# YoungYoung619/road-object-detection-for-bdd100k

Measured on AMD Instinct MI355X. Metric: training images/sec at 1280x720 bf16, higher is better.
Workload: dtype bf16; 1 GPU; REFINE train step (train.py), MobileNet-v2 RefineDet, 720x1280, 8 images/GPU; global_batch=8, train_range=REFINE, parallelism=dp1, augment=False, hip_graph=True, graph_mode=full

## Files before the change

road-object-detection-for-bdd100k_amd/csrc/gemm.hip:

```cpp
#include "rod_common.h"
#include "bnstat_common.h"

namespace rod {

constexpr int BK = 32;

template <typename T> struct LdsPad;
template <> struct LdsPad<bf16_t> { static constexpr int v = 8; };
template <> struct LdsPad<float> { static constexpr int v = 4; };

template <typename T> struct Chunk8;
template <> struct Chunk8<bf16_t> {
  bf16x8 v;
  bool ok;
  __device__ __forceinline__ void zero() {
#pragma unroll
    for (int j = 0; j < 8; ++j) v[j] = (bf16_t)0.f;
    ok = false;
  }
  __device__ __forceinline__ void load_vec(const bf16_t* p) {
    v = *(const bf16x8*)p;
    ok = true;
  }
  __device__ __forceinline__ void set(int j, bf16_t x) { v[j] = x; }
// ... 1218 lines not shown
    __syncthreads();
  }
  const int K = KS * KS * Cin;
  const int tid = threadIdx.x, lane = tid & 63, wave = tid >> 6;
  const int wm = wave >> 1, wn = wave & 1;
  int tile = blockIdx.x, split = blockIdx.y;
  if (gridDim.x > 1 && (gridDim.y & 7) == 0) {
    const long pl = blockIdx.x + (long)blockIdx.y * gridDim.x;
    const long q = pl >> 3;
    tile = (int)(q % gridDim.x);
    split = (int)((q / gridDim.x) * 8 + (pl & 7));
  }
  const int co0 = (tile / ktiles) * WG_T;
  const int k0 = (tile % ktiles) * WG_T;
  const long mb = (long)split * chunk;
  const long me = mb + chunk < M ? mb + chunk : M;

  const int lr = tid >> 3;
  const int lc = (tid & 7) * 8;

  f32x4 acc[2][2];
#pragma unroll
  for (int a = 0; a < 2; ++a)
#pragma unroll
    for (int b = 0; b < 2; ++b)
#pragma unroll
      for (int r = 0; r < 4; ++r) acc[a][b][r] = 0.f;

  Chunk8<T> rdv[RPT], rxv[RPT];
  constexpr bool WALKW = KS == 3 && VA && CIN == 0;
  int wy[RPT], wx[RPT], wnn[RPT], kdy = 0, kdx = 0, kci = 0;
  bool kok = false;
  if constexpr (WALKW) {
    const int kk = k0 + lc;
    kok = kk < K;
    const int tap = kok ? kk / Cin : 0;
    kci = kk - tap * Cin;
    kdy = tap / 3 - 1;
    kdx = tap % 3 - 1;
#pragma unroll
    for (int u = 0; u < RPT; ++u) {
      const long row = mb + lr + u * BK;
      wx[u] = (int)(row % W);
      const long t = row / W;
      wy[u] = (int)(t % H);
      wnn[u] = (int)(t / H);
    }
  }
  auto load_one = [&](long row, Chunk8<T>& rd, Chunk8<T>& rx) {
    if (row >= me || co0 + lc >= Cout) {
      rd.zero();
    } else if (VD && co0 + lc + 8 <= Cout) {
      rd.load_vec(DY + row * lddy + co0 + lc);
    } else {
#pragma unroll
      for (int j = 0; j < 8; ++j) rd.set(j, (co0 + lc + j < Cout) ? DY[row * lddy + co0 + lc + j] : (T)0.f);
    }
    if constexpr (!WALKW) {
      RowSrc<T, KS, CIN> rs;
      rs.init(X, row < me ? row : M, M, H, W, ldx);
      rs.template load<VA, PRO>(rx, k0 + lc, K, Cin, H, W, ldx, pro_lds, pro.act);
    }
  };
  auto load_step = [&](long m) {
#pragma unroll
    for (int u = 0; u < RPT; ++u) {
      load_one(m + lr + u * BK, rdv[u], rxv[u]);
      if constexpr (WALKW) {
        const long row = m + lr + u * BK;
        const int yy = wy[u] + kdy, xx = wx[u] + kdx;
        if (kok && row < me && yy >= 0 && yy < H && xx >= 0 && xx < W)
          rxv[u].load_vec(X + (((long)wnn[u] * H + yy) * W + xx) * ldx + kci);
        else
          rxv[u].zero();
        wx[u] += RPT * BK;
        while (wx[u] >= W) {
          wx[u] -= W;
          if (++wy[u] == H) {
            wy[u] = 0;
            ++wnn[u];
          }
        }
      }
    }
  };

  if (mb < me) load_step(mb);
  for (long m = mb; m < me; m += RPT * BK) {
    __syncthreads();
#pragma unroll
    for (int u = 0; u < RPT; ++u) {
      rdv[u].store_lds(Ds + (lr + u * BK) * WG_LD + lc);
      if constexpr (PRO && WALKW) {
        if (rxv[u].ok) rxv[u].pro(pro_lds, kci, pro.act);
      } else if constexpr (PRO) {
        RowSrc<T, KS, CIN> rp;
        rp.template pro_pending<PRO>(rxv[u], k0 + lc, Cin, pro_lds, pro.act);
      }
      rxv[u].store_lds(Xs + (lr + u * BK) * WG_LD + lc);
    }
    __syncthreads();
    if (m + RPT * BK < me) load_step(m + RPT * BK);
#pragma unroll
    for (int u = 0; u < RPT; ++u)
    if constexpr (sizeof(T) == 2) {
      const int g = lane >> 4, i = lane & 15, q = i >> 2, p = i & 3;
#pragma unroll
      for (int a = 0; a < 2; ++a) {
        const int cb = wm * 32 + a * 16;
        const bf16x4 lo = tr_read((const bf16_t*)Ds + (u * BK + 8 * g + q) * WG_LD + cb + 4 * p);
        const bf16x4 hi = tr_read((const bf16_t*)Ds + (u * BK + 8 * g + 4 + q) * WG_LD + cb + 4 * p);
        bf16x8 fa = {lo[0], lo[1], lo[2], lo[3], hi[0], hi[1], hi[2], hi[3]};
#pragma unroll
        for (int b = 0; b < 2; ++b) {
          const int kb = wn * 32 + b * 16;
          const bf16x4 l2 = tr_read((const bf16_t*)Xs + (u * BK + 8 * g + q) * WG_LD + kb + 4 * p);
          const bf16x4 h2 = tr_read((const bf16_t*)Xs + (u * BK + 8 * g + 4 + q) * WG_LD + kb + 4 * p);
          bf16x8 fb = {l2[0], l2[1], l2[2], l2[3], h2[0], h2[1], h2[2], h2[3]};
          acc[a][b] = __builtin_amdgcn_mfma_f32_16x16x32_bf16(fa, fb, acc[a][b], 0, 0, 0);
        }
      }
    } else {
      const int i = lane & 15, q = lane >> 4;
#pragma unroll
      for (int kk = 0; kk < BK / 4; ++kk) {
        const int mr = u * BK + kk * 4 + q;
#pragma unroll
        for (int a = 0; a < 2; ++a) {
          const float av = ((const float*)Ds)[mr * WG_LD + wm * 32 + a * 16 + i];
#pragma unroll
          for (int b = 0; b < 2; ++b) {
            const float bv = ((const float*)Xs)[mr * WG_LD + wn * 32 + b * 16 + i];
            acc[a][b] = __builtin_amdgcn_mfma_f32_16x16x4f32(av, bv, acc[a][b], 0, 0, 0);
          }
        }
      }
    }
  }
  float* out = part + (long)split * Cout * K;
#pragma unroll
  for (int a = 0; a < 2; ++a)
#pragma unroll
    for (int b = 0; b < 2; ++b) {
      const int k = k0 + wn * 32 + b * 16 + (lane & 15);
      if (k >= K) continue;
#pragma unroll
      for (int r = 0; r < 4; ++r) {
        const int co = co0 + wm * 32 + a * 16 + (lane >> 4) * 4 + r;
        if (co < Cout) out[(long)co * K + k] = acc[a][b][r];
      }
    }
}


struct StemWgradPlan {
  int xb, yb, rb, nblk;
};
static StemWgradPlan stem_wgrad_plan(int N, int H, int W) {
  StemWgradPlan p;
  p.xb = cdiv(W, SW_TW);
  const long segs = (long)N * H * p.xb;
  p.rb = (int)std::max<long>(1, cdivl(segs, 2048));
  p.yb = cdiv(H, p.rb);
  p.nblk = N * p.yb * p.xb;
  return p;
}

struct StemBnb {
  const bf16_t* dz;
  const bf16_t* y;
  const float *mean, *rstd, *gamma, *beta, *coef;
  int act;
};
template <bool BNB>
__global__ void __launch_bounds__(256) stem_wgrad_kernel(const bf16_t* __restrict__ X, const bf16_t* __restrict__ DY,
                                                         float* __restrict__ part, int H, int W, int ldx, int lddy,
                                                         int rb, StemBnb bb) {
  __shared__ __attribute__((aligned(16))) bf16_t lds[2 * SW_TW * SW_LD];
  bf16_t* Ds = lds;
  bf16_t* Xs = lds + SW_TW * SW_LD;
  const int tid = threadIdx.x, lane = tid & 63, wave = tid >> 6;
  const int x0 = blockIdx.x * SW_TW;
  const int n = blockIdx.z;
  const int ya = blockIdx.y * rb;
  const int yz = ya + rb < H ? ya + rb : H;
  const int px = BNB ? tid >> 2 : tid >> 1, half = tid & 1, ck = tid & 3;
  const int xx = x0 + px;
  const bool inx = xx < W, inx2 = xx + 64 < W;
  const int pg = tid & 127, hg = tid >> 7;
  float sc[BNB ? 8 : 1], sh[BNB ? 8 : 1], ca[BNB ? 8 : 1], k1[BNB ? 8 : 1], k0[BNB ? 8 : 1];
  float ghi = 0.f, glo = 0.f;
  if constexpr (BNB) {
#pragma unroll
    for (int e = 0; e < 8; ++e) {
      const int c = ck * 8 + e;
      bn_affine(bb.mean, bb.rstd, bb.gamma, bb.beta, c, sc[e], sh[e]);
      ca[e] = bb.coef[c];
      bn_bwd_k_fold(ca[e], bb.mean[c], bb.rstd[c], bb.coef[32 + c], bb.coef[64 + c], k1[e], k0[e]);
    }
    ghi = bb.act == ROD_ACT_RELU6 ? 6.f : INFINITY;
    glo = bb.act == ROD_ACT_LEAKY ? 0.2f : bb.act == ROD_ACT_NONE ? 1.f : 0.f;
  }
  auto apply = [&](const bf16x8& dzv, const bf16x8& yv) {
    bf16x8 o;
#pragma unroll
    for (int e = 0; e < 8; ++e) {
      const float yj = (float)yv[e];
      const float z = fmaf(yj, sc[e], sh[e]);
      const float gj = (float)dzv[e] * (z > 0.f ? (z < ghi ? 1.f : 0.f) : glo);
      o[e] = (bf16_t)bn_bwd_apply1<bf16_t>(ca[e], gj, k1[e], k0[e], 0.f, yj);
    }
    return o;
  };

  bf16x8 d0, d1, y0, y1;
  unsigned short tv[16];
  const unsigned short* Xu = (const unsigned short*)X;
  auto load_row = [&](int y) {
#pragma unroll
    for (int j = 0; j < 8; ++j) d0[j] = d1[j] = y0[j] = y1[j] = (bf16_t)0.f;
    if constexpr (BNB) {
      const long r = ((long)n * H + y) * W;
      if (inx) {
        d0 = *(const bf16x8*)(bb.dz + (r + xx) * 32 + ck * 8);
        y0 = *(const bf16x8*)(bb.y + (r + xx) * 32 + ck * 8);
      }
      if (inx2) {
        d1 = *(const bf16x8*)(bb.dz + (r + xx + 64) * 32 + ck * 8);
        y1 = *(const bf16x8*)(bb.y + (r + xx + 64) * 32 + ck * 8);
      }
    } else if (inx) {
      const bf16_t* src = DY + (((long)n * H + y) * W + xx) * lddy + half * 16;
      d0 = *(const bf16x8*)src;
      d1 = *(const bf16x8*)(src + 8);
    }
    if (hg) stem_gather<1>(Xu, (long)n * H, y, x0 + pg, H, W, ldx, tv);
    else stem_gather<0>(Xu, (long)n * H, y, x0 + pg, H, W, ldx, tv);
  };

  f32x4 acc[2][2];
#pragma unroll
  for (int a = 0; a < 2; ++a)
#pragma unroll
    for (int b = 0; b < 2; ++b)
#pragma unroll
      for (int r = 0; r < 4; ++r) acc[a][b][r] = 0.f;

  if (ya < yz) load_row(ya);
  for (int y = ya; y < yz; ++y) {
    __syncthreads();
    if constexpr (BNB) {
      bf16x8 z8;
#pragma unroll
      for (int j = 0; j < 8; ++j) z8[j] = (bf16_t)0.f;
      *(bf16x8*)(Ds + px * SW_LD + ck * 8) = inx ? apply(d0, y0) : z8;
      *(bf16x8*)(Ds + (px + 64) * SW_LD + ck * 8) = inx2 ? apply(d1, y1) : z8;
    } else {
      *(bf16x8*)(Ds + px * SW_LD + half * 16) = d0;
      *(bf16x8*)(Ds + px * SW_LD + half * 16 + 8) = d1;
    }
    {
      typedef unsigned short u16x8 __attribute__((ext_vector_type(8)));
      u16x8 t0, t1;
#pragma unroll
      for (int j = 0; j < 8; ++j) {
        t0[j] = tv[j];
        t1[j] = tv[8 + j];
      }
      *(u16x8*)(Xs + pg * SW_LD + hg * 16) = t0;
      *(u16x8*)(Xs + pg * SW_LD + hg * 16 + 8) = t1;
    }
    __syncthreads();
    if (y + 1 < yz) load_row(y + 1);
    const int g = lane >> 4, i = lane & 15, q = i >> 2, p = i & 3;
    const int m0 = wave * 32;
#pragma unroll
    for (int a = 0; a < 2; ++a) {
      const bf16x4 lo = tr_read(Ds + (m0 + 8 * g + q) * SW_LD + a * 16 + 4 * p);
      const bf16x4 hi = tr_read(Ds + (m0 + 8 * g + 4 + q) * SW_LD + a * 16 + 4 * p);
      bf16x8 fa = {lo[0], lo[1], lo[2], lo[3], hi[0], hi[1], hi[2], hi[3]};
#pragma unroll
      for (int b = 0; b < 2; ++b) {
        const bf16x4 l2 = tr_read(Xs + (m0 + 8 * g + q) * SW_LD + b * 16 + 4 * p);
        const bf16x4 h2 = tr_read(Xs + (m0 + 8 * g + 4 + q) * SW_LD + b * 16 + 4 * p);
        bf16x8 fb = {l2[0], l2[1], l2[2], l2[3], h2[0], h2[1], h2[2], h2[3]};
        acc[a][b] = __builtin_amdgcn_mfma_f32_16x16x32_bf16(fa, fb, acc[a][b], 0, 0, 0);
      }
    }
  }
  __syncthreads();
  float* red = (float*)lds;
#pragma unroll
  for (int a = 0; a < 2; ++a)
#pragma unroll
    for (int b = 0; b < 2; ++b)
#pragma unroll
      for (int r = 0; r < 4; ++r) {
        const int co = a * 16 + (lane >> 4) * 4 + r, k = b * 16 + (lane & 15);
        red[(wave * 32 + co) * 32 + k] = acc[a][b][r];
      }
  __syncthreads();
  const long blk = ((long)n * gridDim.y + blockIdx.y) * gridDim.x + blockIdx.x;
  float* out = part + blk * 32 * 27;
  for (int e = tid; e < 32 * 27; e += 256) {
    const int co = e / 27, k = e - co * 27;
    float s = red[co * 32 + k];
    s += red[(32 + co) * 32 + k];
    s += red[(64 + co) * 32 + k];
    s += red[(96 + co) * 32 + k];
    out[e] = s;
  }
}

__global__ void split_reduce_kernel(const float* __restrict__ part, float* __restrict__ out, int splits, long n) {
  long i = (long)blockIdx.x * blockDim.x + threadIdx.x;
  if (i >= n) return;
  float s = 0.f;
  for (int b = 0; b < splits; ++b) s += part[(long)b * n + i];
  out[i] = s;
}

template <typename T>
__global__ void __launch_bounds__(256) colsum_kernel(const T* __restrict__ dy, long M, int C, int ld, long chunk,
                                                     float* __restrict__ slab) {
  __shared__ float red[256];
  const int tid = threadIdx.x;
  const int CB = C < 256 ? C : 256;
  const int lanes = 256 / CB;
  const int cl = tid % CB, ln = tid / CB;
  const int c = blockIdx.y * 256 + cl;
  const long r0 = (long)blockIdx.x * chunk;
  const long r1 = r0 + chunk < M ? r0 + chunk : M;
  float s0 = 0.f, s1 = 0.f, s2 = 0.f, s3 = 0.f;
  if (ln < lanes && c < C) {
    long r = r0 + ln;
    for (; r + 3L * lanes < r1; r += 4L * lanes) {
      s0 += to_f32(dy[r * ld + c]);
      s1 += to_f32(dy[(r + lanes) * ld + c]);
      s2 += to_f32(dy[(r + 2L * lanes) * ld + c]);
      s3 += to_f32(dy[(r + 3L * lanes) * ld + c]);
    }
    for (; r < r1; r += lanes) s0 += to_f32(dy[r * ld + c]);
  }
  red[tid] = (s0 + s1) + (s2 + s3);
  __syncthreads();
  if (ln == 0 && c < C) {
    float t = 0.f;
    for (int l = 0; l < lanes; ++l) t += red[l * CB + cl];
    slab[(long)blockIdx.x * C + c] = t;
  }
}

template <typename T>
__global__ void weight_prep_kernel(const float* __restrict__ w, T* __restrict__ wt, int Cout, int Cin, int ks,
                                   int mode) {
  const long n = (long)Cout * ks * ks * Cin;
  long idx = (long)blockIdx.x * blockDim.x + threadIdx.x;
  if (idx >= n) return;
  if (mode == 0) {
    wt[idx] = from_f32<T>(w[idx]);
    return;
  }
  const int co = (int)(idx % Cout);
  long t = idx / Cout;
  const int j = (int)(t % ks);
  t /= ks;
  const int i = (int)(t % ks);
  const int ci = (int)(t / ks);
  const int si = ks - 1 - i, sj = ks - 1 - j;
  wt[idx] = from_f32<T>(w[(((long)co * ks + si) * ks + sj) * Cin + ci]);
}

struct PrepEntry {
  const float* w;
  void* wt;
  long start;
  int Cout, Cin, ksize, mode;
};
static_assert(sizeof(PrepEntry) == 40, "rod_prep_entry layout");

template <typename T>
__global__ void __launch_bounds__(256) weight_prep_batch_kernel(const PrepEntry* __restrict__ tab, int n, long total) {
  for (long idx = (long)blockIdx.x * blockDim.x + threadIdx.x; idx < total; idx += (long)gridDim.x * blockDim.x) {
    int lo = 0, hi = n - 1;
    while (lo < hi) {
      const int mid = (lo + hi + 1) >> 1;
      if (tab[mid].start <= idx) lo = mid;
      else hi = mid - 1;
    }
    const PrepEntry e = tab[lo];
    const long i = idx - e.start;
    T* wt = (T*)e.wt;
    if (e.mode == 0) {
      wt[i] = from_f32<T>(e.w[i]);
      continue;
    }
    const int co = (int)(i % e.Cout);
    long t = i / e.Cout;
    const int j = (int)(t % e.ksize);
    t /= e.ksize;
    const int ii = (int)(t % e.ksize);
    const int ci = (int)(t / e.ksize);
    wt[i] = from_f32<T>(e.w[(((long)co * e.ksize + (e.ksize - 1 - ii)) * e.ksize + (e.ksize - 1 - j)) * e.Cin + ci]);
  }
}

struct WgradPlan {
  int ctiles, ktiles, splits;
  long chunk;
};
static WgradPlan wgrad_plan(long M, int Cin, int Cout, int ks) {
  WgradPlan p;
  const int K = ks * ks * Cin;
  p.ctiles = cdiv(Cout, WG_T);
  p.ktiles = cdiv(K, WG_T);
  const int tiles = p.ctiles * p.ktiles;
  constexpr long WG_TARGET = 2048;
  constexpr long WG_MINROWS = 128;
  long splits = std::max<long>(1, std::min<long>(cdivl(WG_TARGET, tiles), cdivl(M, WG_MINROWS)));
  long chunk = cdivl(M, splits);
  chunk = cdivl(chunk, BK) * BK;
  p.chunk = chunk;
  p.splits = (int)cdivl(M, chunk);
  if (tiles > 1 && p.splits >= 8) p.splits = (p.splits + 7) / 8 * 8;
  return p;
}

template <typename T>
static bool aligned16(const void* p) {
  return ((uintptr_t)p & 15) == 0;
}

template <typename T, int KS, int BN, bool VA, bool VB, bool VY, bool PRO>
static void conv_fwd_launch(const void* x, const void* wt, const float* bias, void* y, long M, int H, int W, int Cin,
                            int Cout, int ldx, int ldy, float* stats, const BnPro& pro, const BnGred* gr,
                            hipStream_t s, const BnEpi* ep = nullptr, const BnBwd* bw = nullptr) {
  dim3 grid(cdivl(M, 128), cdiv(Cout, BN));
  if (grid.y > 1) grid.x = (grid.x + 7) / 8 * 8;
  const size_t lds = PRO ? 8 * (size_t)Cin : 0;
  if constexpr (sizeof(T) == 2 && KS == 1 && !PRO && VA) {
    if (bw) {
      hipLaunchKernelGGL((conv_fwd_kernel<T, KS, BN, VA, VB, VY, false, false, false, false, false, true>), grid,
                         dim3(256), (size_t)Cin * BWD_CF * sizeof(float), s, (const T*)x, (const T*)wt, bias, (T*)y, M,
                         H, W, Cin, Cout, ldx, ldy, nullptr, 0, pro, BnGred{}, BnEpi{}, *bw);
      return;
    }
  }
  if constexpr (sizeof(T) == 2) {
    if (ep) {
      hipLaunchKernelGGL((conv_fwd_kernel<T, KS, BN, VA, VB, VY, false, false, PRO, false, true>), grid,
                         dim3(256), lds, s, (const T*)x, (const T*)wt, bias, (T*)y, M, H, W, Cin, Cout, ldx, ldy,
                         nullptr, 0, pro, BnGred{}, *ep);
      return;
    }
  }
  if constexpr (VY) {
    if (gr) {
      hipLaunchKernelGGL((conv_fwd_kernel<T, KS, BN, VA, VB, VY, false, false, PRO, true>), grid, dim3(256), lds, s,
                         (const T*)x, (const T*)wt, bias, (T*)y, M, H, W, Cin, Cout, ldx, ldy, nullptr, 0, pro, *gr);
      return;
    }
    if (stats) {
      hipLaunchKernelGGL((conv_fwd_kernel<T, KS, BN, VA, VB, VY, false, true, PRO, false>), grid, dim3(256), lds, s,
                         (const T*)x, (const T*)wt, bias, (T*)y, M, H, W, Cin, Cout, ldx, ldy, stats, 0, pro);
      return;
    }
  }
  hipLaunchKernelGGL((conv_fwd_kernel<T, KS, BN, VA, VB, VY, false, false, PRO, false>), grid, dim3(256), lds, s,
                     (const T*)x, (const T*)wt, bias, (T*)y, M, H, W, Cin, Cout, ldx, ldy, nullptr, 0, pro);
}

template <typename T, int KS, bool PRO>
static void conv_fwd_dispatch(bool va, bool vb, bool vy, const void* x, const void* wt, const float* bias, void* y,
                              long M, int H, int W, int Cin, int Cout, int ldx, int ldy, float* stats,
                              const BnPro& pro, const BnGred* gr, hipStream_t s, const BnEpi* ep = nullptr,
                              const BnBwd* bw = nullptr) {
  auto cf = [&](auto BN_, auto VA_, auto VY_) {
    conv_fwd_launch<T, KS, BN_, VA_, VY_, VY_, PRO>(x, wt, bias, y, M, H, W, Cin, Cout, ldx, ldy, stats, pro, gr, s, ep,
                                                    bw);
  };
  if (va && vb && vy) {
    const int bn = Cout <= 192 ? cdiv(Cout, 32) * 32 : Cout <= 256 ? 256 : 128;
    sel_int<32, 64, 96, 128, 160, 192, 256>(bn, [&](auto BN_) { cf(BN_, std::true_type{}, std::true_type{}); });
    return;
  }
  const int bn = Cout <= 96 ? cdiv(Cout, 32) * 32 : 128;
  sel_int<32, 64, 96, 128>(bn, [&](auto BN_) {
    sel_bool(va, [&](auto VA_) { cf(BN_, VA_, std::false_type{}); });
  });
}

template <typename T, int KS, bool PRO, bool VA, bool VB>
static void conv_fwd_split_t(const SplitPlan& p, const void* x, const void* wt, float* part, long M, int H, int W,
                             int Cin, int Cout, int ldx, const BnPro& pro, hipStream_t s, const BnBwd* bw = nullptr) {
  dim3 grid(cdivl(M, 128), cdiv(Cout, 128), p.splits);
  const size_t lds = PRO ? 8 * (size_t)Cin : 0;
  if constexpr (sizeof(T) == 2 && KS == 1 && !PRO && VA) {
    if (bw) {
      hipLaunchKernelGGL((conv_fwd_kernel<T, KS, 128, VA, VB, false, true, false, false, false, false, true>), grid,
                         dim3(256), (size_t)Cin * BWD_CF * sizeof(float), s, (const T*)x, (const T*)wt, nullptr,
                         nullptr, M, H, W, Cin, Cout, ldx, 0, part, p.kper, pro, BnGred{}, BnEpi{}, *bw);
      return;
    }
  }
  hipLaunchKernelGGL((conv_fwd_kernel<T, KS, 128, VA, VB, false, true, false, PRO>), grid, dim3(256), lds, s,
                     (const T*)x, (const T*)wt, nullptr, nullptr, M, H, W, Cin, Cout, ldx, 0, part, p.kper, pro);
}
template <typename T, int KS, bool PRO>
static void conv_fwd_split(bool va, bool vb, const SplitPlan& p, const void* x, const void* wt, float* part, long M,
                           int H, int W, int Cin, int Cout, int ldx, const BnPro& pro, hipStream_t s,
                           const BnBwd* bw = nullptr) {
  if (va && vb) conv_fwd_split_t<T, KS, PRO, true, true>(p, x, wt, part, M, H, W, Cin, Cout, ldx, pro, s, bw);
  else if (va) conv_fwd_split_t<T, KS, PRO, true, false>(p, x, wt, part, M, H, W, Cin, Cout, ldx, pro, s, bw);
  else if (vb) conv_fwd_split_t<T, KS, PRO, false, true>(p, x, wt, part, M, H, W, Cin, Cout, ldx, pro, s);
  else conv_fwd_split_t<T, KS, PRO, false, false>(p, x, wt, part, M, H, W, Cin, Cout, ldx, pro, s);
}

template <typename T>
static void conv_fwd_typed(const void* x, const BnPro* pro, const void* wt, const float* bias, void* y, void* ws,
                           float* stats, const BnGred* gr, int N, int H, int W, int Cin, int Cout, int ksize, int ldx,
                           int ldy, hipStream_t s, const BnEpi* ep = nullptr, const BnBwd* bw = nullptr) {
  const long M = (long)N * H * W;
  const int K = ksize * ksize * Cin;
  const int eV = Vec16<T>::N;
  const bool va = aligned16<T>(x) && (ldx % eV == 0) && (ksize == 1 ? true : (Cin % 8 == 0));
  const bool vb = aligned16<T>(wt) && (K % eV == 0);
  const bool vy = aligned16<T>(y) && (ldy % eV == 0);
  const SplitPlan sp = split_plan(M, Cout, K);
  const int nparts = (int)cdivl(M, 128);
  const int dt = sizeof(T) == 4 ? ROD_F32 : ROD_BF16;
  const BnPro pv = pro ? *pro : BnPro{};
  if constexpr (sizeof(T) == 2) {
    if (!pro && !gr && !ep && !bw && ksize == 3 && Cin == 3 && Cout == 32 && vy) {
      const bool fuse = stats != nullptr && W % SW_TW == 0;
      const int xb = cdiv(W, SW_TW);
      const int rb = (int)std::max<long>(1, std::min<long>(8, (long)N * H * xb / 8192));
      const dim3 grid(xb, cdiv(H, rb), N);
      if (fuse)
        hipLaunchKernelGGL(stem_fwd_mfma_kernel<true>, grid, dim3(256), 0, s, (const bf16_t*)x, (const bf16_t*)wt,
                           bias, (bf16_t*)y, stats, H, W, ldx, ldy, rb);
      else
        hipLaunchKernelGGL(stem_fwd_mfma_kernel<false>, grid, dim3(256), 0, s, (const bf16_t*)x, (const bf16_t*)wt,
                           bias, (bf16_t*)y, nullptr, H, W, ldx, ldy, rb);
      if (stats && !fuse) stat_parts(dt, y, M, Cout, ldy, stats, nparts, s);
      return;
    }
  }
  if (ws != nullptr && sp.splits > 1 && !(ksize == 3 && Cin == 3)) {
    float* part = (float*)ws;
    if (ksize == 1) {
      if (pro) conv_fwd_split<T, 1, true>(va, vb, sp, x, wt, part, M, H, W, Cin, Cout, ldx, pv, s);
      else conv_fwd_split<T, 1, false>(va, vb, sp, x, wt, part, M, H, W, Cin, Cout, ldx, pv, s, bw);
    } else {
      if (pro) conv_fwd_split<T, 3, true>(va, vb, sp, x, wt, part, M, H, W, Cin, Cout, ldx, pv, s);
      else conv_fwd_split<T, 3, false>(va, vb, sp, x, wt, part, M, H, W, Cin, Cout, ldx, pv, s);
    }
    if (ep)
      hipLaunchKernelGGL((splitk_combine_kernel<T, true>), dim3(cdivl(M * Cout, 256)), dim3(256), 0, s,
                         (const float*)part, bias, (T*)y, M, Cout, ldy, sp.splits, *ep);
    else
      hipLaunchKernelGGL(splitk_combine_kernel<T>, dim3(cdivl(M * Cout, 256)), dim3(256), 0, s, (const float*)part,
                         bias, (T*)y, M, Cout, ldy, sp.splits);
    if (stats) stat_parts(dt, y, M, Cout, ldy, stats, nparts, s);
    if (gr) gred_parts(dt, y, gr->y, gr->p, M, Cout, gr->parts, nparts, s);
    return;
  }
  if ((stats || gr) && !(va && vb && vy)) {
    conv_fwd_typed<T>(x, pro, wt, bias, y, ws, nullptr, nullptr, N, H, W, Cin, Cout, ksize, ldx, ldy, s);
    if (stats) stat_parts(dt, y, M, Cout, ldy, stats, nparts, s);
    if (gr) gred_parts(dt, y, gr->y, gr->p, M, Cout, gr->parts, nparts, s);
    return;
  }
  if (!pro && !gr && !ep && ksize == 3 && Cin == 3 && vy) {
    if constexpr (sizeof(T) == 4) {
      if (Cout == 32) {
        hipLaunchKernelGGL((stem_conv_fwd_kernel<T, 32>), dim3(cdiv(W, 128), H, N), dim3(256), 0, s, (const T*)x,
                           (const T*)wt, bias, (T*)y, H, W, ldx, ldy);
        return;
      }
    }
    if (Cout == 64) {
      hipLaunchKernelGGL((stem_conv_fwd_kernel<T, 64>), dim3(cdiv(W, 64), H, N), dim3(256), 0, s, (const T*)x,
                         (const T*)wt, bias, (T*)y, H, W, ldx, ldy);
      return;
    }
  }
  if constexpr (sizeof(T) == 2) {
    if (!ep && !bw && !gr && pro && ksize == 1 && !bias && va && vb && vy && Cin <= PRO_MAXC &&
        pw_proj_launch((const bf16_t*)x, (const bf16_t*)wt, (bf16_t*)y, M, K, Cout, ldx, ldy, stats, s, pv))
      return;
    if (!ep && !bw && ksize == 1 && !bias && va && vb && vy && (!pro || (K <= 32 && Cin <= PRO_MAXC)) &&
        pw_stream_launch((const bf16_t*)x, (const bf16_t*)wt, (bf16_t*)y, M, K, Cout, ldx, ldy, stats, gr, s,
                         pro ? &pv : nullptr))
      return;
  }
  if (ksize == 1) {
    if (pro) conv_fwd_dispatch<T, 1, true>(va, vb, vy, x, wt, bias, y, M, H, W, Cin, Cout, ldx, ldy, stats, pv, gr, s, ep);
    else conv_fwd_dispatch<T, 1, false>(va, vb, vy, x, wt, bias, y, M, H, W, Cin, Cout, ldx, ldy, stats, pv, gr, s, ep,
                                        bw);
  } else {
    if (pro) conv_fwd_dispatch<T, 3, true>(va, vb, vy, x, wt, bias, y, M, H, W, Cin, Cout, ldx, ldy, stats, pv, gr, s, ep);
    else conv_fwd_dispatch<T, 3, false>(va, vb, vy, x, wt, bias, y, M, H, W, Cin, Cout, ldx, ldy, stats, pv, gr, s, ep);
  }
}

template <typename T, int KS, bool VA, bool VD, bool PRO>
static void wgrad_launch(const WgradPlan& p, const void* x, const void* dy, float* part, long M, int H, int W,
                         int Cin, int Cout, int ldx, int lddy, const BnPro& pro, hipStream_t s) {
  dim3 grid(p.ctiles * p.ktiles, p.splits);
  const size_t lds = PRO ? 8 * (size_t)Cin : 0;
  hipLaunchKernelGGL((conv_wgrad_kernel<T, KS, VA, VD, 0, PRO>), grid, dim3(256), lds, s, (const T*)x, (const T*)dy,
                     part, M, H, W, Cin, Cout, ldx, lddy, p.chunk, p.ktiles, pro);
}

template <typename T, int KS, bool PRO>
static void wgrad_va_vd(bool va, bool vd, const WgradPlan& p, const void* x, const void* dy, float* part, long M,
                        int H, int W, int Cin, int Cout, int ldx, int lddy, const BnPro& pro, hipStream_t s) {
  if (va && vd) wgrad_launch<T, KS, true, true, PRO>(p, x, dy, part, M, H, W, Cin, Cout, ldx, lddy, pro, s);
  else if (va) wgrad_launch<T, KS, true, false, PRO>(p, x, dy, part, M, H, W, Cin, Cout, ldx, lddy, pro, s);
  else if (vd) wgrad_launch<T, KS, false, true, PRO>(p, x, dy, part, M, H, W, Cin, Cout, ldx, lddy, pro, s);
  else wgrad_launch<T, KS, false, false, PRO>(p, x, dy, part, M, H, W, Cin, Cout, ldx, lddy, pro, s);
}

static long wgrad_part_floats(int N, int H, int W, int Cin, int Cout, int ksize) {
  const long M = (long)N * H * W;
  WgradPlan p = wgrad_plan(M, Cin, Cout, ksize);
  const long K = (long)ksize * ksize * Cin;
  if (ksize == 3 && Cin == 3 && Cout == 32) p.splits = std::max(p.splits, stem_wgrad_plan(N, H, W).nblk);
  return ((long)p.splits * Cout * K + 3) / 4 * 4;
}

template <typename T>
static void wgrad_typed(const void* x, const BnPro* pro, const void* dy, float* dw, float* db, float* part, int N,
                        int H, int W, int Cin, int Cout, int ksize, int ldx, int lddy, hipStream_t s) {
  const long M = (long)N * H * W;
  const long K = (long)ksize * ksize * Cin;
  WgradPlan p = wgrad_plan(M, Cin, Cout, ksize);
  const int eV = Vec16<T>::N;
  const bool va = aligned16<T>(x) && (ldx % eV == 0) && (ksize == 1 ? true : (Cin % 8 == 0));
  const bool vd = aligned16<T>(dy) && (lddy % eV == 0);
  const BnPro pv = pro ? *pro : BnPro{};
  bool stem = false;
  if constexpr (sizeof(T) == 2) {
    if (!pro && ksize == 3 && Cin == 3 && Cout == 32 && vd) {
      const StemWgradPlan sp = stem_wgrad_plan(N, H, W);
      hipLaunchKernelGGL(stem_wgrad_kernel<false>, dim3(sp.xb, sp.yb, N), dim3(256), 0, s, (const bf16_t*)x,
                         (const bf16_t*)dy, part, H, W, ldx, lddy, sp.rb, StemBnb{});
      p.splits = sp.nblk;
      stem = true;
    }
  }
  if (stem) {
  } else if (!pro && ksize == 3 && Cin == 3 && vd) {
    dim3 grid(p.ctiles * p.ktiles, p.splits);
    hipLaunchKernelGGL((conv_wgrad_kernel<T, 3, false, true, 3>), grid, dim3(256), 0, s, (const T*)x, (const T*)dy,
                       part, M, H, W, Cin, Cout, ldx, lddy, p.chunk, p.ktiles, pv);
  } else if (ksize == 1) {
    if (pro) wgrad_va_vd<T, 1, true>(va, vd, p, x, dy, part, M, H, W, Cin, Cout, ldx, lddy, pv, s);
    else wgrad_va_vd<T, 1, false>(va, vd, p, x, dy, part, M, H, W, Cin, Cout, ldx, lddy, pv, s);
  } else {
    if (pro) wgrad_va_vd<T, 3, true>(va, vd, p, x, dy, part, M, H, W, Cin, Cout, ldx, lddy, pv, s);
    else wgrad_va_vd<T, 3, false>(va, vd, p, x, dy, part, M, H, W, Cin, Cout, ldx, lddy, pv, s);
  }
  const long n = (long)Cout * K;
  slab_sum(part, dw, p.splits, n, s);
  if (db) {
    long cchunk = std::max<long>(64, cdivl(M, 512));
    int nb = (int)cdivl(M, cchunk);
    float* partb = part + wgrad_part_floats(N, H, W, Cin, Cout, ksize);
    hipLaunchKernelGGL(colsum_kernel<T>, dim3(nb, cdiv(Cout, 256)), dim3(256), 0, s, (const T*)dy, M, Cout, lddy,
                       cchunk, partb);
    slab_sum(partb, db, nb, (long)Cout, s);
  }
}

}

using namespace rod;

extern "C" {

int rod_conv_fwd_stream_ok(long M, int K, int Cout, int dtype) {
  int nt = 0;
  return dtype == ROD_BF16 && pw_stream_groups(M, K, Cout, nt) > 0 ? 1 : 0;
}

size_t rod_conv_fwd_workspace(int N, int H, int W, int Cin, int Cout, int ksize) {
  const long M = (long)N * H * W;
  const SplitPlan p = split_plan(M, Cout, ksize * ksize * Cin);
  return p.splits > 1 ? (size_t)p.splits * M * Cout * sizeof(float) : 0;
}

int rod_conv_fwd(const void* x, const float* pro_mean, const float* pro_rstd, const float* pro_gamma,
                 const float* pro_beta, int pro_act, const void* wt, const float* bias, void* y, void* workspace,
                 float* stat_parts, const void* gred_y, const float* gred_mean, const float* gred_rstd,
                 const float* gred_gamma, const float* gred_beta, int gred_act, float* gred_parts, int N, int H, int W,
                 int Cin, int Cout, int ksize, int ldx, int ldy, int dtype, void* stream) {
  ROD_CHECK_ARG(N > 0 && H > 0 && W > 0 && Cin > 0 && Cout > 0, "rod_conv_fwd: bad shape");
  ROD_CHECK_ARG(ksize == 1 || ksize == 3, "rod_conv_fwd: ksize must be 1 or 3");
  if (ldx == 0) ldx = Cin;
  if (ldy == 0) ldy = Cout;
  ROD_CHECK_ARG(ldx >= Cin && ldy >= Cout, "rod_conv_fwd: leading dim too small");
  ROD_CHECK_ARG(!pro_mean || (pro_rstd && Cin <= PRO_MAXC), "rod_conv_fwd: bad BatchNorm prologue (Cin %d)", Cin);
  ROD_CHECK_ARG(!gred_parts || (gred_y && gred_mean && gred_rstd && ldy == Cout && !stat_parts),
                "rod_conv_fwd: gred needs y, mean, rstd, a dense output and no stat_parts");
  const BnPro pro{pro_mean, pro_rstd, pro_gamma, pro_beta, pro_act};
  const BnGred gr{gred_y, BnPro{gred_mean, gred_rstd, gred_gamma, gred_beta, gred_act}, gred_parts};
  auto run = [&](auto tag) {
    typedef decltype(tag) T;
    conv_fwd_typed<T>(x, pro_mean ? &pro : nullptr, wt, bias, y, workspace, stat_parts, gred_parts ? &gr : nullptr, N,
                      H, W, Cin, Cout, ksize, ldx, ldy, ROD_STREAM(stream));
  };
  ROD_CHECK_ARG(sel_dtype(dtype, run), "rod_conv_fwd: unsupported dtype code %d", dtype);
  return check_launch("rod_conv_fwd");
}

int rod_conv_fwd_stats_supported(long M, int Cin, int Cout, int dtype) {
  int nt = 0;
  return dtype == ROD_BF16 && Cin <= 32 && pw_stream_groups(M, Cin, Cout, nt, false) > 0 ? 1 : 0;
}

int rod_conv_fwd_stats(const void* x, const float* pro_mean, const float* pro_rstd, const float* pro_gamma,
                       const float* pro_beta, int pro_act, const void* wt, float* stat_parts, long M, int Cin, int Cout,
                       int dtype, void* stream) {
  ROD_CHECK_ARG(rod_conv_fwd_stats_supported(M, Cin, Cout, dtype),
                "rod_conv_fwd_stats: unsupported M=%ld Cin=%d Cout=%d dtype=%d", M, Cin, Cout, dtype);
  ROD_CHECK_ARG(x && wt && stat_parts, "rod_conv_fwd_stats: NULL argument");
  ROD_CHECK_ARG(!pro_mean || pro_rstd, "rod_conv_fwd_stats: bad BatchNorm prologue");
  ROD_CHECK_ARG(((((uintptr_t)x) | ((uintptr_t)wt)) & 15) == 0, "rod_conv_fwd_stats: x, wt must be 16-byte aligned");
  const BnPro pro{pro_mean, pro_rstd, pro_gamma, pro_beta, pro_act};
  if (!pw_stream_launch((const bf16_t*)x, (const bf16_t*)wt, nullptr, M, Cin, Cout, Cin, Cout, stat_parts, nullptr,
                        ROD_STREAM(stream), pro_mean ? &pro : nullptr)) {
    set_error("rod_conv_fwd_stats: no statistics-only plan for M=%ld Cin=%d Cout=%d", M, Cin, Cout);
    return ROD_EINVAL;
  }
  return check_launch("rod_conv_fwd_stats");
}

int rod_conv_fwd_bnact(const void* x, const float* pro_mean, const float* pro_rstd, const float* pro_gamma,
                       const float* pro_beta, int pro_act, const void* wt, const float* bias, void* z, void* workspace,
                       const float* bn_mean, const float* bn_rstd, const float* bn_gamma, const float* bn_beta,
                       int bn_act, const void* res, int ldr, int N, int H, int W, int Cin, int Cout, int ksize,
                       int ldx, int ldy, int dtype, void* stream) {
  ROD_CHECK_ARG(N > 0 && H > 0 && W > 0 && Cin > 0 && Cout > 0, "rod_conv_fwd_bnact: bad shape");
  ROD_CHECK_ARG(ksize == 1 || ksize == 3, "rod_conv_fwd_bnact: ksize must be 1 or 3");
  ROD_CHECK_ARG(dtype == ROD_BF16, "rod_conv_fwd_bnact: bf16 only (dtype %d)", dtype);
  ROD_CHECK_ARG(bn_mean && bn_rstd && z, "rod_conv_fwd_bnact: BatchNorm mean / rstd and the output required");
  ROD_CHECK_ARG(bn_act >= ROD_ACT_NONE && bn_act <= ROD_ACT_RELU, "rod_conv_fwd_bnact: bad act %d", bn_act);
  if (ldx == 0) ldx = Cin;
  if (ldy == 0) ldy = Cout;
  if (ldr == 0) ldr = Cout;
  ROD_CHECK_ARG(ldx >= Cin && ldy >= Cout && (!res || ldr >= Cout), "rod_conv_fwd_bnact: leading dim too small");
  ROD_CHECK_ARG(!res || (((uintptr_t)res & 15) == 0 && ldr % 8 == 0), "rod_conv_fwd_bnact: res 16-byte rows");
  ROD_CHECK_ARG(!pro_mean || (pro_rstd && Cin <= PRO_MAXC), "rod_conv_fwd_bnact: bad BatchNorm prologue (Cin %d)", Cin);
  const BnPro pro{pro_mean, pro_rstd, pro_gamma, pro_beta, pro_act};
  const BnEpi ep{bn_mean, bn_rstd, bn_gamma, bn_beta, res, ldr, bn_act};
  conv_fwd_typed<bf16_t>(x, pro_mean ? &pro : nullptr, wt, bias, z, workspace, nullptr, nullptr, N, H, W, Cin, Cout,
                         ksize, ldx, ldy, ROD_STREAM(stream), &ep);
  return check_launch("rod_conv_fwd_bnact");
}

constexpr int BWD_STATIC_LDS = 32 * 1024;
static int bwd_data_bn_max_cout() {
  static int cached = -1;
  if (cached < 0) {
    int dev = 0, lds = 0;
    if (hipGetDevice(&dev) != hipSuccess ||
        hipDeviceGetAttribute(&lds, hipDeviceAttributeMaxSharedMemoryPerBlock, dev) != hipSuccess || lds <= 0)
      lds = 64 * 1024;
    cached = (lds - BWD_STATIC_LDS) / (BWD_CF * (int)sizeof(float)) / 8 * 8;
  }
  return cached;
}

int rod_conv_bwd_data_bn_supported(int Cout, int Cin, int dtype) {
  return dtype == ROD_BF16 && Cout % 8 == 0 && Cin % 8 == 0 && Cout > 0 && Cout <= bwd_data_bn_max_cout() ? 1 : 0;
}

int rod_conv_bwd_data_bn(const void* dz, const void* y, const float* mean, const float* rstd, const float* gamma,
                         const float* beta, int act, const float* coef, const void* wt1, void* dy, void* dx,
                         void* workspace, long M, int Cout, int Cin, int dtype, void* stream) {
  ROD_CHECK_ARG(M > 0 && rod_conv_bwd_data_bn_supported(Cout, Cin, dtype),
                "rod_conv_bwd_data_bn: unsupported M=%ld Cout=%d Cin=%d dtype=%d", M, Cout, Cin, dtype);
  ROD_CHECK_ARG(dz && y && mean && rstd && coef && wt1 && dy && dx, "rod_conv_bwd_data_bn: NULL argument");
  ROD_CHECK_ARG(act >= ROD_ACT_NONE && act <= ROD_ACT_RELU, "rod_conv_bwd_data_bn: bad act %d", act);
  ROD_CHECK_ARG(((((uintptr_t)dz) | ((uintptr_t)y) | ((uintptr_t)wt1) | ((uintptr_t)dy) | ((uintptr_t)dx)) & 15) == 0,
                "rod_conv_bwd_data_bn: tensors must be 16-byte aligned");
  ROD_CHECK_ARG(M <= 0x7fffffffL, "rod_conv_bwd_data_bn: M too large");
  const BnBwd bw{(const bf16_t*)y, mean, rstd, gamma, beta, coef, act, (bf16_t*)dy};
  conv_fwd_typed<bf16_t>(dz, nullptr, wt1, nullptr, dx, workspace, nullptr, nullptr, 1, 1, (int)M, Cout, Cin, 1, Cout,
                         Cin, ROD_STREAM(stream), nullptr, &bw);
  return check_launch("rod_conv_bwd_data_bn");
}
// ... 79 lines not shown
```

road-object-detection-for-bdd100k_amd/rod/roofline.py:

```python

_ES = {0: 4, 1: 2}

COST_MODEL_VERSION = 2

MI355X_HBM_PEAK_GBS = 8000.0
MI355X_BF16_PEAK_TFLOPS = 2500.0
MI355X_F32_PEAK_TFLOPS = 157.3


def box_iou_loss_bytes(B, A, es, n_pos, grad=True):
    return B * A * (4 + (4 * es if grad else 0)) + n_pos * (8 * es + 32)


def cost(name, a):
    if name == "rod_augment_images":
        B, Ho, Wo, dt = a[8], a[9], a[10], a[12]
        return (_ES[dt] + 1) * B * Ho * Wo * 3, 0
    if name == "rod_mosaic_images":
        B, Ho, Wo, dt = a[11], a[12], a[13], a[15]
        return (_ES[dt] + 1) * B * Ho * Wo * 3, 0
    if name == "rod_dw3x3_fwd":
        N, H, W, C, Ho, Wo, dt = a[9], a[10], a[11], a[12], a[16], a[17], a[18]
        es = _ES[dt]
        return es * (N * H * W * C + N * Ho * Wo * C) + 36 * C, 18 * N * Ho * Wo * C
# ... 87 lines not shown
        es = _ES[dt]
        want_dx = a[15] is not None
        byts = es * (M * Cout + M * Cin + (M * Cin if want_dx else 0)) + Cout * Cin * (2 * es + 4)
        return byts, 2 * M * Cin * Cout * (3 if want_dx else 2) + 10 * M * Cout
    if name == "rod_pw_bwd_gred_rc":
        M, Cin, Cout, dt = a[19], a[20], a[21], a[22]
        es = _ES[dt]
        return es * (M * Cout + 2 * M * Cin) + Cout * Cin * (2 * es + 4), \
            6 * M * Cin * Cout + 10 * M * Cout + 6 * M * Cin
    if name == "rod_pw_bwd_gred_dyp":
        M, Cin, Cout, dt = a[19], a[20], a[21], a[22]
        es = _ES[dt]
        return es * (3 * M * Cout + M * Cin) + Cout * Cin * (es + 4), \
            4 * M * Cin * Cout + 10 * M * Cout + 6 * M * Cin
    if name == "rod_ir_block_fwd":
        N, H, W, Cin, inner, Cout, s, dt = a[18], a[19], a[20], a[21], a[22], a[23], a[24], a[25]
        es = _ES[dt]
        Ho, Wo = -(-H // s), -(-W // s)
        byts = es * (N * H * W * Cin + N * Ho * Wo * Cout) + es * inner * (Cin + Cout) + 36 * inner
        return byts, 2 * N * H * W * Cin * inner + 18 * N * Ho * Wo * inner + 2 * N * Ho * Wo * inner * Cout
    if name == "rod_match_anchors":
        B, A, G = a[12], a[13], a[14]
        return B * A * 56 + A * 32 + B * G * 20, 15 * G * A * B
    if name == "rod_normalize_image":
        n, dt = a[2], a[3]
        return (1 + _ES[dt]) * n, 2 * n
    if name == "rod_cast":
        n = a[4]
        return (_ES[a[1]] + _ES[a[3]]) * n, 0
    if name == "rod_bn_stat_parts":
        M, C, nparts, dt = a[1], a[2], a[4], a[5]
        return _ES[dt] * M * C + 12 * nparts * C, 3 * M * C
    if name == "rod_bn_finalize":
        nparts, C = a[1], a[3]
        return 12 * nparts * C + 16 * C, 10 * nparts * C
    if name == "rod_bn_bwd_parts":
        M, C, nparts, dt = a[9], a[10], a[8], a[11]
        return _ES[dt] * M * C * 2 + 8 * nparts * C, 6 * M * C
    if name == "rod_bn_bwd_finalize":
        nparts, C = a[1], a[3]
        return 8 * nparts * C + 24 * C, 4 * nparts * C
    if name == "rod_bn_eval_stats":
        C = a[5]
        return 16 * C, 3 * C
    if name == "rod_copy2d":
        return 2 * a[4] * a[5], 0
    if name == "rod_add":
        n, dt = a[3], a[4]
        return 3 * _ES[dt] * n, n
    if name == "rod_sgd_clip":
        n = a[2]
        return 12 * n, 3 * n
    if name == "rod_sgd_momentum":
        n, mom = a[4], a[2] is not None
        return (20 if mom else 12) * n + n // 4, 9 * n
    if name == "rod_sgd_momentum_ema":
        n, mom = a[5], a[2] is not None
        return (28 if mom else 20) * n + n // 4, 12 * n
    if name == "rod_grad_sqnorm":
        n = a[2]
        return 4 * n + n // 4, 2 * n
    if name == "rod_conv_weight_prep_batch":
        total, dt = a[2], a[3]
        return (4 + _ES[dt]) * total, 0
    if name == "rod_smoothl1_masked":
        B, A, dt = a[10], a[11], a[12]
        es = _ES[dt]
        wgt = a[8] is not None
        return B * A * (4 * es + 16 + 4 + 4 * es + (16 if wgt else 0)), 12 * B * A * 4
    if name == "rod_box_iou_loss":
        B, A, dt = a[13], a[14], a[15]
        return box_iou_loss_bytes(B, A, _ES[dt], B * A, a[11] is not None), 80 * B * A
    if name == "rod_decode":
        B, A, dt = a[4], a[5], a[7]
        return B * A * (2 * 4 * _ES[dt] + 16) + 16 * A, 20 * B * A
    if name == "rod_softmax":
        rows, K, dt = a[2], a[3], a[4]
        return rows * K * (_ES[dt] + 4), 4 * rows * K
    if name in ("rod_softmax_focal", "rod_focal_loss"):
        off = 0 if name == "rod_softmax_focal" else 1
        B, A, K, dt = a[8 + off], a[9 + off], a[10 + off], a[11 + off]
        g = a[6 + off] is not None
        return B * A * (K * _ES[dt] * (2 if g else 1) + (12 - 4 * off)), 60 * B * A * K
    if name == "rod_focal_count":
        return 4 * a[3] * a[4], a[3] * a[4]
    if name == "rod_select_topk_nms":
        B, A, K = a[2], a[3], a[4]
        return B * A * (K * 4 + 16), 0
    if name == "rod_select_topk_softnms":
        B, A, K, top_k, keep = a[2], a[3], a[4], a[6], a[7]
        return B * A * (K * 4 + 16), 25 * B * (K - 1) * keep * min(top_k, A)
    if name == "rod_det_targets":
        B, A, dt = a[13], a[14], a[15]
        return B * A * (4 * _ES[dt] + 16 + 16 + 4 + 4 + 16 + 4 + 4 + 4), 40 * B * A
    if name in ("rod_resize_bilinear", "rod_resize_bilinear_bwd"):
        N, H, W, C, Ho, Wo, dt = a[2], a[3], a[4], a[5], a[6], a[7], a[8]
        return _ES[dt] * C * N * (H * W + Ho * Wo), 8 * N * Ho * Wo * C
    if name in ("rod_depth_to_space2", "rod_space_to_depth2"):
        N, h, w, Fc, dt = a[2], a[3], a[4], a[5], a[9]
        return 2 * _ES[dt] * N * h * w * 4 * Fc, 0
    return 0, 0


def design_bytes(name, a):
    if name == "rod_bn_bwd_apply":
        M, C, dt = a[8], a[9], a[11]
        return _ES[dt] * M * C * 3
    if name == "rod_dw3x3_bwd_fused":
        N, C, Ho, Wo, dt = a[19], a[22], a[26], a[27], a[28]
        return cost(name, a)[0] + _ES[dt] * 2 * N * Ho * Wo * C
    if name == "rod_dw3x3_bwd_fused_rc":
        N, C, Ho, Wo, dt = a[26], a[29], a[33], a[34], a[35]
        return cost(name, a)[0] + _ES[dt] * 2 * N * Ho * Wo * C
    if name == "rod_dw3x3_bwd_fused_pw":
        N, H, W, C, dt, cout = a[21], a[22], a[23], a[24], a[25], a[8]
        return cost(name, a)[0] + _ES[dt] * N * H * W * (C + cout)
    return cost(name, a)[0]


def kernel_match(name, pat):
    inc, *exc = pat.split('!')
    return all(t in name for t in inc.split('&')) and not any(t in name for t in exc)


_PW = ('2, 3, true>', 'Li2ELi3ELb1EE')
_BWD = ('32, false, true>', 'Li32ELb0ELb1EE')
_XG = (', true, true, true, ', 'Lb1ELb1ELb1E')
_LAST = ('true>(rod::PwBwdArgs', 'Lb1EEEvNS_9PwBwdArgs')
_STATS_ONLY = (', 1, 3', 'ELi1ELi3E')


def _forms(base, inc=(), exc=()):
    heads = ('rod::%s<' % base, '_ZN3rod%d%sI' % (len(base), base))
    return tuple('&'.join([heads[i]] + [t[i] for t in inc]) + ''.join('!' + t[i] for t in exc) for i in (0, 1))

ENTRY_KERNELS = {
    "rod_bn_bwd": (("bn_bwd_small_kernel",), ("bn_bwd_small_kernel",)),
    "rod_bn_apply": (("bn_apply_kernel",), ("bn_apply_kernel",)),
    "rod_bn_bwd_reduce": (("bn_bwd_reduce_kernel",), ("bn_bwd_reduce_kernel", "bn_bwd_finalize_kernel")),
    "rod_bn_bwd_apply": (("bn_bwd_apply_kernel",), ("bn_bwd_apply_kernel",)),
    "rod_pw_bwd": (_forms("pw_bwd_kernel") + _forms("pw_bwd_stream_kernel", exc=(_XG, _LAST)),) * 2,
    "rod_pw_bwd_rc": (_forms("pw_bwd_stream_kernel", inc=(_LAST,), exc=(_XG,)),) * 2,
    "rod_pw_bwd_gred": (_forms("pw_bwd_gred_kernel", exc=(_LAST,)) +
                        _forms("pw_bwd_stream_kernel", inc=(_XG,), exc=(_LAST,)),) * 2,
    "rod_pw_bwd_gred_rc": (_forms("pw_bwd_stream_kernel", inc=(_XG, _LAST)),) * 2,
    "rod_pw_bwd_gred_dyp": (_forms("pw_bwd_gred_kernel", inc=(_LAST,)),) * 2,
    "rod_dw3x3_fwd": (("dw3x3_fwd_!dw3x3_fwd_rc",), ("dw3x3_fwd_!dw3x3_fwd_rc",)),
    "rod_dw3x3_fwd_rc": (("dw3x3_fwd_rc_kernel",), ("dw3x3_fwd_rc_kernel",)),
    "rod_dw3x3_bwd_data": (("dw3x3_bwd_data",), ("dw3x3_bwd_data",)),
    "rod_dw3x3_bwd_filter": (("dw3x3_bwdw_lx", "dw3x3_bwd_filter_kernel"), ("dw3x3_bwdw_lx", "dw3x3_bwd_filter_kernel")),
    "rod_dw3x3_bwd_fused": (("dw3x3_bwd_fused!dw3x3_bwd_fused_rc!" + "!".join(_PW),),) * 2,
    "rod_dw3x3_bwd_fused_rc": (("dw3x3_bwd_fused_rc_kernel",),) * 2,
    "rod_dw3x3_bwd_fused_pw": tuple(tuple("dw3x3_bwd_fused2&" + t for t in _PW) for _ in range(2)),
    "rod_conv_wgrad": (("conv_wgrad_kernel",), ("conv_wgrad_kernel", "colsum_kernel")),
    "rod_conv_fwd": (("conv_fwd_kernel!" + "!".join(_BWD), "stem_fwd_mfma_kernel") +
                     _forms("pw_stream_kernel", exc=(_STATS_ONLY,)),) * 2,
    "rod_conv_fwd_stats": (_forms("pw_stream_kernel", inc=(_STATS_ONLY,)),) * 2,
    "rod_conv_bwd_data_bn": tuple(tuple("conv_fwd_kernel&" + t for t in _BWD) for _ in range(2)),
    "rod_bn_finalize": (("bn_parts_merge_kernel",), ("bn_parts_merge_kernel",)),
    "rod_ir_block_fwd": (("ir_block_fwd_kernel",), ("ir_block_fwd_kernel",)),
}
```

Before: 484.3 images/s.

## Add 128x128-tile wide weight-gradient kernel with fewer split-K partials for large convs

Adds a bf16 conv weight-gradient kernel that uses 128x128 output tiles (4x4 MFMA fragments per wave) instead of the smaller generic tile, with its own split planner that targets about two resident blocks per CU. It is selected for aligned layers with K>=64 and Cout>=96. The aim is more operand reuse per LDS load and fewer split-K partial buffers to write and reduce. In exchange it uses more registers and LDS per block, so occupancy drops, and it provides fewer blocks for parallelism. The roofline kernel map is updated to include the new kernel.

```diff
diff --git a/road-object-detection-for-bdd100k_amd/csrc/gemm.hip b/road-object-detection-for-bdd100k_amd/csrc/gemm.hip
--- a/road-object-detection-for-bdd100k_amd/csrc/gemm.hip
+++ b/road-object-detection-for-bdd100k_amd/csrc/gemm.hip
@@ -1394,6 +1394,166 @@
     }
 }
 
+constexpr int WW_T = 128;
+constexpr int WW_LD = WW_T + 16;
+constexpr int WW_LDS_BYTES = 2 * 2 * BK * WW_LD * 2;
+constexpr int WW_RESIDENT = 2;
+
+template <int KS, bool PRO>
+__global__ void __launch_bounds__(256) conv_wgrad_wide_kernel(const bf16_t* __restrict__ X,
+                                                              const bf16_t* __restrict__ DY,
+                                                              float* __restrict__ part, long M, int H, int W,
+                                                              int Cin, int Cout, int ldx, int lddy, long chunk,
+                                                              int ktiles, BnPro pro = BnPro{}) {
+  typedef bf16_t T;
+  __shared__ __attribute__((aligned(16))) T Ds[2][BK * WW_LD];
+  __shared__ __attribute__((aligned(16))) T Xs[2][BK * WW_LD];
+  extern __shared__ float pro_lds[];
+  if constexpr (PRO) {
+    stage_pro(pro_lds, pro, Cin);
+    __syncthreads();
+  }
+  const int K = KS * KS * Cin;
+  const int tid = threadIdx.x, lane = tid & 63, wave = tid >> 6;
+  const int wm = wave >> 1, wn = wave & 1;
+  int tile = blockIdx.x, split = blockIdx.y;
+  if (gridDim.x > 1 && (gridDim.y & 7) == 0) {
+    const long pl = blockIdx.x + (long)blockIdx.y * gridDim.x;
+    const long q = pl >> 3;
+    tile = (int)(q % gridDim.x);
+    split = (int)((q / gridDim.x) * 8 + (pl & 7));
+  }
+  const int co0 = (tile / ktiles) * WW_T;
+  const int k0 = (tile % ktiles) * WW_T;
+  const long mb = (long)split * chunk;
+  const long me = mb + chunk < M ? mb + chunk : M;
+  const int nsteps = mb < me ? (int)((me - mb + BK - 1) / BK) : 0;
+
+  const int lr = tid >> 4;
+  const int lc = (tid & 15) * 8;
+
+  f32x4 acc[4][4];
+#pragma unroll
+  for (int a = 0; a < 4; ++a)
+#pragma unroll
+    for (int b = 0; b < 4; ++b)
+#pragma unroll
+      for (int r = 0; r < 4; ++r) acc[a][b][r] = 0.f;
+
+  Chunk8<T> rdv[2], rxv[2];
+  int wy[2], wx[2], wnn[2], kdy = 0, kdx = 0, kci = 0;
+  bool kok = false;
+  if constexpr (KS == 3) {
+    const int kk = k0 + lc;
+    kok = kk < K;
+    const int tap = kok ? kk / Cin : 0;
+    kci = kk - tap * Cin;
+    kdy = tap / 3 - 1;
+    kdx = tap % 3 - 1;
+#pragma unroll
+    for (int u = 0; u < 2; ++u) {
+      const long row = mb + lr + u * 16;
+      wx[u] = (int)(row % W);
+      const long t = row / W;
+      wy[u] = (int)(t % H);
+      wnn[u] = (int)(t / H);
+    }
+  }
+  auto load_step = [&](long m) {
+#pragma unroll
+    for (int u = 0; u < 2; ++u) {
+      const long row = m + lr + u * 16;
+      if (row >= me || co0 + lc >= Cout) {
+        rdv[u].zero();
+      } else if (co0 + lc + 8 <= Cout) {
+        rdv[u].load_vec(DY + row * lddy + co0 + lc);
+      } else {
+#pragma unroll
+        for (int j = 0; j < 8; ++j) rdv[u].set(j, (co0 + lc + j < Cout) ? DY[row * lddy + co0 + lc + j] : (T)0.f);
+      }
+      if constexpr (KS == 1) {
+        RowSrc<T, 1> rs;
+        rs.init(X, row < me ? row : M, M, H, W, ldx);
+        rs.template load<true, PRO>(rxv[u], k0 + lc, K, Cin, H, W, ldx, pro_lds, pro.act);
+      } else {
+        const int yy = wy[u] + kdy, xx = wx[u] + kdx;
+        if (kok && row < me && yy >= 0 && yy < H && xx >= 0 && xx < W)
+          rxv[u].load_vec(X + (((long)wnn[u] * H + yy) * W + xx) * ldx + kci);
+        else
+          rxv[u].zero();
+        wx[u] += BK;
+        while (wx[u] >= W) {
+          wx[u] -= W;
+          if (++wy[u] == H) {
+            wy[u] = 0;
+            ++wnn[u];
+          }
+        }
+      }
+    }
+  };
+  auto stage = [&](int buf) {
+#pragma unroll
+    for (int u = 0; u < 2; ++u) {
+      rdv[u].store_lds(Ds[buf] + (lr + u * 16) * WW_LD + lc);
+      if constexpr (PRO && KS == 3) {
+        if (rxv[u].ok) rxv[u].pro(pro_lds, kci, pro.act);
+      } else if constexpr (PRO) {
+        RowSrc<T, 1> rp;
+        rp.template pro_pending<PRO>(rxv[u], k0 + lc, Cin, pro_lds, pro.act);
+      }
+      rxv[u].store_lds(Xs[buf] + (lr + u * 16) * WW_LD + lc);
+    }
+  };
+
+  if (nsteps > 0) {
+    load_step(mb);
+    stage(0);
+    if (nsteps > 1) load_step(mb + BK);
+    __syncthreads();
+  }
+  const int g = lane >> 4, i = lane & 15, q = i >> 2, p = i & 3;
+  const int fo = (4 * g + q) * WW_LD + 4 * p;
+  for (int st = 0; st < nsteps; ++st) {
+    const int cur = st & 1;
+    if (st + 1 < nsteps) {
+      stage(cur ^ 1);
+      if (st + 2 < nsteps) load_step(mb + (long)(st + 2) * BK);
+    }
+    const T* dsb = Ds[cur] + fo + wm * 64;
+    const T* xsb = Xs[cur] + fo + wn * 64;
+    bf16x8 fb[4];
+#pragma unroll
+    for (int b = 0; b < 4; ++b) {
+      const bf16x4 lo = tr_read(xsb + b * 16);
+      const bf16x4 hi = tr_read(xsb + 16 * WW_LD + b * 16);
+      fb[b] = bf16x8{lo[0], lo[1], lo[2], lo[3], hi[0], hi[1], hi[2], hi[3]};
+    }
+#pragma unroll
+    for (int a = 0; a < 4; ++a) {
+      const bf16x4 lo = tr_read(dsb + a * 16);
+      const bf16x4 hi = tr_read(dsb + 16 * WW_LD + a * 16);
+      const bf16x8 fa = {lo[0], lo[1], lo[2], lo[3], hi[0], hi[1], hi[2], hi[3]};
+#pragma unroll
+      for (int b = 0; b < 4; ++b) acc[a][b] = __builtin_amdgcn_mfma_f32_16x16x32_bf16(fa, fb[b], acc[a][b], 0, 0, 0);
+    }
+    __syncthreads();
+  }
+  float* out = part + (long)split * Cout * K;
+#pragma unroll
+  for (int a = 0; a < 4; ++a)
+#pragma unroll
+    for (int b = 0; b < 4; ++b) {
+      const int k = k0 + wn * 64 + b * 16 + (lane & 15);
+      if (k >= K) continue;
+#pragma unroll
+      for (int r = 0; r < 4; ++r) {
+        const int co = co0 + wm * 64 + a * 16 + (lane >> 4) * 4 + r;
+        if (co < Cout) out[(long)co * K + k] = acc[a][b][r];
+      }
+    }
+}
+
 
 struct StemWgradPlan {
   int xb, yb, rb, nblk;
@@ -1650,10 +1810,12 @@
 struct WgradPlan {
   int ctiles, ktiles, splits;
   long chunk;
+  bool wide;
 };
-static WgradPlan wgrad_plan(long M, int Cin, int Cout, int ks) {
+static WgradPlan wgrad_plan_generic(long M, int Cin, int Cout, int ks) {
   WgradPlan p;
   const int K = ks * ks * Cin;
+  p.wide = false;
   p.ctiles = cdiv(Cout, WG_T);
   p.ktiles = cdiv(K, WG_T);
   const int tiles = p.ctiles * p.ktiles;
@@ -1665,6 +1827,29 @@
   p.chunk = chunk;
   p.splits = (int)cdivl(M, chunk);
   if (tiles > 1 && p.splits >= 8) p.splits = (p.splits + 7) / 8 * 8;
+  return p;
+}
+static bool wgrad_wide_shape(long M, int Cin, int Cout, int ks) {
+  return ks * ks * Cin >= 64 && Cout >= 96;
+}
+static WgradPlan wgrad_plan(long M, int Cin, int Cout, int ks, bool wide_ok = false) {
+  const WgradPlan gp = wgrad_plan_generic(M, Cin, Cout, ks);
+  if (!wide_ok || !wgrad_wide_shape(M, Cin, Cout, ks)) return gp;
+  WgradPlan p;
+  const int K = ks * ks * Cin;
+  p.wide = true;
+  p.ctiles = cdiv(Cout, WW_T);
+  p.ktiles = cdiv(K, WW_T);
+  const int tiles = p.ctiles * p.ktiles;
+  constexpr long WW_BLOCKS = 256 * WW_RESIDENT;
+  constexpr long WW_MINROWS = 128;
+  long want = std::max<long>(1, std::min<long>(cdivl(WW_BLOCKS, tiles), cdivl(M, WW_MINROWS)));
+  want = std::min<long>(want, gp.splits);
+  const bool xcd = tiles > 1 && want >= 8;
+  if (xcd) want = want / 8 * 8;
+  p.chunk = cdivl(cdivl(M, want), BK) * BK;
+  p.splits = (int)cdivl(M, p.chunk);
+  if (xcd) p.splits = (p.splits + 7) / 8 * 8;
   return p;
 }
 
@@ -1858,6 +2043,15 @@
 template <typename T, int KS, bool PRO>
 static void wgrad_va_vd(bool va, bool vd, const WgradPlan& p, const void* x, const void* dy, float* part, long M,
                         int H, int W, int Cin, int Cout, int ldx, int lddy, const BnPro& pro, hipStream_t s) {
+  if constexpr (sizeof(T) == 2) {
+    if (p.wide) {
+      dim3 grid(p.ctiles * p.ktiles, p.splits);
+      hipLaunchKernelGGL((conv_wgrad_wide_kernel<KS, PRO>), grid, dim3(256), PRO ? 8 * (size_t)Cin : 0, s,
+                         (const bf16_t*)x, (const bf16_t*)dy, part, M, H, W, Cin, Cout, ldx, lddy, p.chunk, p.ktiles,
+                         pro);
+      return;
+    }
+  }
   if (va && vd) wgrad_launch<T, KS, true, true, PRO>(p, x, dy, part, M, H, W, Cin, Cout, ldx, lddy, pro, s);
   else if (va) wgrad_launch<T, KS, true, false, PRO>(p, x, dy, part, M, H, W, Cin, Cout, ldx, lddy, pro, s);
   else if (vd) wgrad_launch<T, KS, false, true, PRO>(p, x, dy, part, M, H, W, Cin, Cout, ldx, lddy, pro, s);
@@ -1877,10 +2071,10 @@
                         int H, int W, int Cin, int Cout, int ksize, int ldx, int lddy, hipStream_t s) {
   const long M = (long)N * H * W;
   const long K = (long)ksize * ksize * Cin;
-  WgradPlan p = wgrad_plan(M, Cin, Cout, ksize);
   const int eV = Vec16<T>::N;
   const bool va = aligned16<T>(x) && (ldx % eV == 0) && (ksize == 1 ? true : (Cin % 8 == 0));
   const bool vd = aligned16<T>(dy) && (lddy % eV == 0);
+  WgradPlan p = wgrad_plan(M, Cin, Cout, ksize, sizeof(T) == 2 && va && vd);
   const BnPro pv = pro ? *pro : BnPro{};
   bool stem = false;
   if constexpr (sizeof(T) == 2) {
diff --git a/road-object-detection-for-bdd100k_amd/rod/roofline.py b/road-object-detection-for-bdd100k_amd/rod/roofline.py
--- a/road-object-detection-for-bdd100k_amd/rod/roofline.py
+++ b/road-object-detection-for-bdd100k_amd/rod/roofline.py
@@ -263,7 +263,8 @@
     "rod_dw3x3_bwd_fused": (("dw3x3_bwd_fused!dw3x3_bwd_fused_rc!" + "!".join(_PW),),) * 2,
     "rod_dw3x3_bwd_fused_rc": (("dw3x3_bwd_fused_rc_kernel",),) * 2,
     "rod_dw3x3_bwd_fused_pw": tuple(tuple("dw3x3_bwd_fused2&" + t for t in _PW) for _ in range(2)),
-    "rod_conv_wgrad": (("conv_wgrad_kernel",), ("conv_wgrad_kernel", "colsum_kernel")),
+    "rod_conv_wgrad": (("conv_wgrad_kernel", "conv_wgrad_wide_kernel"),
+                       ("conv_wgrad_kernel", "conv_wgrad_wide_kernel", "colsum_kernel")),
     "rod_conv_fwd": (("conv_fwd_kernel!" + "!".join(_BWD), "stem_fwd_mfma_kernel") +
                      _forms("pw_stream_kernel", exc=(_STATS_ONLY,)),) * 2,
     "rod_conv_fwd_stats": (_forms("pw_stream_kernel", inc=(_STATS_ONLY,)),) * 2,
```

Measured after the change: 485.7 images/s (median of 3 runs). Within noise of the previous version (+0.3%).
